# microsoft/NOTSOFAR1-Challenge

Hardware: AMD Instinct MI355X
Metric: CSS real-time-factor (sep. audio sec/wall sec) on 7-ch 16 kHz (higher is better)
Workload: dtype f32 (float32 operands on v_mfma_f32_32x32x2_f32 in every Linear layer, attention product and transform: the reference's own operand precision; MVDR covariance / solve f64)

## Files before the change

notsofar1-challenge_amd/csrc/encoder.hip:

```cpp
#include "kernels.hpp"
#include "split_f16.hpp"
#include "wave.hpp"

namespace css {

typedef float f32x16 __attribute__((ext_vector_type(16)));
typedef _Float16 f16x8 __attribute__((ext_vector_type(8)));

template <int NV>
__device__ __forceinline__ float ln_centre(float4 (&v)[NV]) {
    constexpr int D = 256 * NV;
    float s = 0.f;
#pragma unroll
    for (int i = 0; i < NV; ++i) s += (v[i].x + v[i].y) + (v[i].z + v[i].w);
    const float mean = wave_sum_dpp(s) * (1.0f / D);
    float q = 0.f;
#pragma unroll
    for (int i = 0; i < NV; ++i) {
        v[i].x -= mean; v[i].y -= mean; v[i].z -= mean; v[i].w -= mean;
        q += (v[i].x * v[i].x + v[i].y * v[i].y) + (v[i].z * v[i].z + v[i].w * v[i].w);
    }
    return 1.0f / sqrtf(wave_sum_dpp(q) * (1.0f / D) + 1e-5f);
}

#ifndef CSS_LN_ROWS
#define CSS_LN_ROWS 4
#endif
constexpr int LN_ROWS = CSS_LN_ROWS;
template <int NV, int MODE>
__global__ __launch_bounds__(64 * LN_ROWS) void layernorm_kernel(const float* __restrict__ x, float* __restrict__ y,
                                                        float* __restrict__ ys, const float* __restrict__ w,
                                                        const float* __restrict__ b, const float* __restrict__ pw,
                                                        int rows) {
    constexpr int D = 256 * NV;
    const int row = blockIdx.x * LN_ROWS + (threadIdx.x >> 6);
    if (row >= rows) return;
    const int lane = threadIdx.x & 63;
    const float4* xr = reinterpret_cast<const float4*>(x + (int64_t)row * D);
    float4 v[NV];
#pragma unroll
    for (int i = 0; i < NV; ++i) v[i] = xr[lane + 64 * i];
    const float rstd = ln_centre(v);
    float p0 = 0.f, p1 = 0.f, p2 = 0.f, p3 = 0.f;
    if (MODE == 2) { p0 = pw[0]; p1 = pw[1]; p2 = pw[2]; p3 = pw[3]; }
    float4* yr = reinterpret_cast<float4*>(y + (int64_t)row * D);
    _Float16* ysr = reinterpret_cast<_Float16*>(ys + (int64_t)row * D);
#pragma unroll
    for (int i = 0; i < NV; ++i) {
        const float4 g = reinterpret_cast<const float4*>(w)[lane + 64 * i];
        const float4 be = reinterpret_cast<const float4*>(b)[lane + 64 * i];
        float o[4] = {v[i].x * rstd * g.x + be.x, v[i].y * rstd * g.y + be.y, v[i].z * rstd * g.z + be.z,
                      v[i].w * rstd * g.w + be.w};
#pragma unroll
        for (int e = 0; e < 4; ++e) {
            if (MODE == 1) o[e] = fmaxf(o[e], 0.f);
            if (MODE == 2) o[e] = (p0 * o[e] + p1) * (1.0f / (1.0f + expf(-(p2 * o[e] + p3))));
        }
        if (y) yr[lane + 64 * i] = make_float4(o[0], o[1], o[2], o[3]);
        if (ys) split_store4(ysr, 4 * (lane + 64 * i), o[0], o[1], o[2], o[3]);
    }
}

template <int NV>
__global__ __launch_bounds__(64 * LN_ROWS) void layernorm2_kernel(const float* __restrict__ x, float* __restrict__ y,
                                                         const float* __restrict__ w1, const float* __restrict__ b1,
                                                         float* __restrict__ z, float* __restrict__ zs,
                                                         const float* __restrict__ w2, const float* __restrict__ b2,
                                                         int rows) {
    constexpr int D = 256 * NV;
    const int row = blockIdx.x * LN_ROWS + (threadIdx.x >> 6);
    if (row >= rows) return;
    const int lane = threadIdx.x & 63;
    const float4* xr = reinterpret_cast<const float4*>(x + (int64_t)row * D);
    float4 v[NV];
#pragma unroll
    for (int i = 0; i < NV; ++i) v[i] = xr[lane + 64 * i];
#pragma unroll
    for (int pass = 0; pass < 2; ++pass) {
        const float rstd = ln_centre(v);
        const float* w = pass ? w2 : w1;
        const float* b = pass ? b2 : b1;
        float* yo = pass ? z : y;
#pragma unroll
        for (int i = 0; i < NV; ++i) {
            const float4 g = reinterpret_cast<const float4*>(w)[lane + 64 * i];
            const float4 be = reinterpret_cast<const float4*>(b)[lane + 64 * i];
            v[i] = make_float4(v[i].x * rstd * g.x + be.x, v[i].y * rstd * g.y + be.y, v[i].z * rstd * g.z + be.z,
                               v[i].w * rstd * g.w + be.w);
            if (yo) reinterpret_cast<float4*>(yo + (int64_t)row * D)[lane + 64 * i] = v[i];
            if (pass && zs)
                split_store4(reinterpret_cast<_Float16*>(zs + (int64_t)row * D), 4 * (lane + 64 * i), v[i].x, v[i].y, v[i].z, v[i].w);
        }
    }
}

void launch_layernorm2(const float* x, float* y, const float* w1, const float* b1, float* z, float* z_split,
                       const float* w2, const float* b2, int rows, int D, hipStream_t s) {
    const dim3 grid((rows + LN_ROWS - 1) / LN_ROWS), block(64 * LN_ROWS);
    switch (D) {
        case 256: hipLaunchKernelGGL((layernorm2_kernel<1>), grid, block, 0, s, x, y, w1, b1, z, z_split, w2, b2, rows); break;
        case 512: hipLaunchKernelGGL((layernorm2_kernel<2>), grid, block, 0, s, x, y, w1, b1, z, z_split, w2, b2, rows); break;
        case 768: hipLaunchKernelGGL((layernorm2_kernel<3>), grid, block, 0, s, x, y, w1, b1, z, z_split, w2, b2, rows); break;
        case 1024: hipLaunchKernelGGL((layernorm2_kernel<4>), grid, block, 0, s, x, y, w1, b1, z, z_split, w2, b2, rows); break;
        default: break;
    }
}

template <int MODE>
static void launch_ln_mode(const float* x, float* y, float* ys, const float* w, const float* b, const float* pw,
                           int rows, int D, hipStream_t s) {
    const dim3 grid((rows + LN_ROWS - 1) / LN_ROWS), block(64 * LN_ROWS);
    switch (D) {
        case 256: hipLaunchKernelGGL((layernorm_kernel<1, MODE>), grid, block, 0, s, x, y, ys, w, b, pw, rows); break;
        case 512: hipLaunchKernelGGL((layernorm_kernel<2, MODE>), grid, block, 0, s, x, y, ys, w, b, pw, rows); break;
        case 768: hipLaunchKernelGGL((layernorm_kernel<3, MODE>), grid, block, 0, s, x, y, ys, w, b, pw, rows); break;
        case 1024: hipLaunchKernelGGL((layernorm_kernel<4, MODE>), grid, block, 0, s, x, y, ys, w, b, pw, rows); break;
        default: break;
    }
}

void launch_layernorm(const float* x, float* y, float* y_split, const float* w, const float* b, int rows, int D,
                      int relu, hipStream_t s) {
    if (relu) launch_ln_mode<1>(x, y, y_split, w, b, nullptr, rows, D, s);
    else launch_ln_mode<0>(x, y, y_split, w, b, nullptr, rows, D, s);
}

void launch_ln_glu(const float* x, float* z, const float* w, const float* b, const float* pw, int rows, int D,
                   hipStream_t s) {
    launch_ln_mode<2>(x, z, nullptr, w, b, pw, rows, D, s);
}

template <int TAPS, int RUN>
__global__ __launch_bounds__(256) void dwconv_kernel(const float* __restrict__ z, float* __restrict__ h,
                                                     const float* __restrict__ wt, const float* __restrict__ dwb,
                                                     const float* __restrict__ alpha, const float* __restrict__ beta,
                                                     const float* __restrict__ pw, int T, int D, int runs_per_seg) {
    constexpr int PAD = (TAPS - 1) / 2;
    const int ch = blockIdx.x * 256 + threadIdx.x;
    if (ch >= D) return;
    const int seg = blockIdx.y / runs_per_seg, run = blockIdx.y % runs_per_seg;
    const int t0 = run * RUN;
    const float* zs = z + (int64_t)seg * T * D + ch;
    float wk[TAPS];
#pragma clang loop unroll(full)
    for (int k = 0; k < TAPS; ++k) wk[k] = wt[k * D + ch];
    float acc[RUN];
#pragma clang loop unroll(full)
    for (int j = 0; j < RUN; ++j) acc[j] = 0.f;
#pragma clang loop unroll(full)
    for (int p = 0; p < RUN + TAPS - 1; ++p) {
        const int t = t0 + p - PAD;
        const float v = (t >= 0 && t < T) ? zs[(int64_t)t * D] : 0.f;
#pragma clang loop unroll(full)
        for (int j = (p - (TAPS - 1) > 0 ? p - (TAPS - 1) : 0); j <= (p < RUN - 1 ? p : RUN - 1); ++j)
            acc[j] = fmaf(wk[p - j], v, acc[j]);
    }
    const float bb = dwb[ch], al = alpha[ch], be = beta[ch], w2 = pw[4], c2 = pw[5];
    float* hs = h + (int64_t)seg * T * D + ch;
#pragma unroll
    for (int j = 0; j < RUN; ++j) {
        const int t = t0 + j;
        if (t < T) {
            const float y = fmaxf((acc[j] + bb) * al + be, 0.f);
            hs[(int64_t)t * D] += w2 * y + c2;
        }
    }
}

void launch_dwconv(const float* z, float* h, const float* dw_wt, const float* dw_b, const float* bn_alpha,
                   const float* bn_beta, const float* pw, int nseg, int T, int D, int taps, hipStream_t s) {
    constexpr int RUN = 31;
    const int runs = (T + RUN - 1) / RUN;
    const dim3 grid((D + 255) / 256, nseg * runs), block(256);
    if (taps == 33)
        hipLaunchKernelGGL((dwconv_kernel<33, RUN>), grid, block, 0, s, z, h, dw_wt, dw_b, bn_alpha, bn_beta, pw, T, D, runs);
    else if (taps == 31)
        hipLaunchKernelGGL((dwconv_kernel<31, RUN>), grid, block, 0, s, z, h, dw_wt, dw_b, bn_alpha, bn_beta, pw, T, D, runs);
    else if (taps == 17)
        hipLaunchKernelGGL((dwconv_kernel<17, RUN>), grid, block, 0, s, z, h, dw_wt, dw_b, bn_alpha, bn_beta, pw, T, D, runs);
}

template <int NV, int TAPS, int RUN, int HV>
__global__ __launch_bounds__(256 * NV * HV) void conv_module_kernel(const float* __restrict__ x_in, float* __restrict__ x_out,
                                                              const float* __restrict__ lnw, const float* __restrict__ lnb,
                                                              const float* __restrict__ pw, const float* __restrict__ wt,
                                                              const float* __restrict__ dwb, const float* __restrict__ alpha,
                                                              const float* __restrict__ beta,
                                                              const float* __restrict__ ln2w, const float* __restrict__ ln2b,
                                                              float* __restrict__ z, float* __restrict__ zs, int T, int runs_per_seg) {
    constexpr int D = 256 * NV, PAD = (TAPS - 1) / 2, ROWS = RUN + TAPS - 1, NW = 4 * NV * HV, JH = (RUN + HV - 1) / HV;
    extern __shared__ __attribute__((aligned(16))) float tile[];
    const int item = css_xcd_item((int)blockIdx.x, (int)gridDim.x);
    const int seg = item / runs_per_seg, run = item % runs_per_seg;
    const int t0 = run * RUN;
    const int wave = threadIdx.x >> 6, lane = threadIdx.x & 63;
    const float p0 = pw[0], p1 = pw[1], p2 = pw[2], p3 = pw[3];
    const int ch = threadIdx.x % D, j0 = (threadIdx.x / D) * JH;
    float wk[TAPS];
#pragma clang loop unroll(full)
    for (int k = 0; k < TAPS; ++k) wk[k] = wt[k * D + ch];
    const float bb = dwb[ch], al = alpha[ch], be_ = beta[ch], w2 = pw[4], c2 = pw[5];
    const float* xs = x_in + (int64_t)seg * T * D + ch;
    float xres[JH];
#pragma clang loop unroll(full)
    for (int j = 0; j < JH; ++j) xres[j] = xs[(int64_t)min(t0 + j0 + j, T - 1) * D];
    constexpr int RPW = (ROWS + NW - 1) / NW;
    float4 v[RPW][NV];
#pragma unroll
    for (int i = 0; i < RPW; ++i) {
        const int p = wave + i * NW, t = t0 + p - PAD;
        const bool ok = p < ROWS && t >= 0 && t < T;
        const float4* xr = reinterpret_cast<const float4*>(x_in + ((int64_t)seg * T + (ok ? t : 0)) * D);
#pragma unroll
        for (int j = 0; j < NV; ++j) v[i][j] = ok ? xr[lane + 64 * j] : make_float4(0.f, 0.f, 0.f, 0.f);
    }
#pragma unroll
    for (int i = 0; i < RPW; ++i) {
        const int p = wave + i * NW, t = t0 + p - PAD;
        if (p >= ROWS) break;
        float4* dst = reinterpret_cast<float4*>(tile + p * D);
        if (t < 0 || t >= T) {
#pragma unroll
            for (int j = 0; j < NV; ++j) dst[lane + 64 * j] = make_float4(0.f, 0.f, 0.f, 0.f);
            continue;
        }
        const float rstd = ln_centre(v[i]);
#pragma unroll
        for (int j = 0; j < NV; ++j) {
            const float4 g = reinterpret_cast<const float4*>(lnw)[lane + 64 * j];
            const float4 be = reinterpret_cast<const float4*>(lnb)[lane + 64 * j];
            float o[4] = {v[i][j].x * rstd * g.x + be.x, v[i][j].y * rstd * g.y + be.y, v[i][j].z * rstd * g.z + be.z,
                          v[i][j].w * rstd * g.w + be.w};
#pragma unroll
            for (int e = 0; e < 4; ++e) {
                const float z = p2 * o[e] + p3;
                o[e] = (p0 * o[e] + p1) * __builtin_amdgcn_rcpf(1.0f + __builtin_amdgcn_exp2f(z * -1.44269504088896341f));
            }
            dst[lane + 64 * j] = make_float4(o[0], o[1], o[2], o[3]);
        }
    }
    __syncthreads();
    float acc[JH];
#pragma clang loop unroll(full)
    for (int j = 0; j < JH; ++j) acc[j] = 0.f;
#pragma clang loop unroll(full)
    for (int pp = 0; pp < JH + TAPS - 1; ++pp) {
        const float zv = tile[min(j0 + pp, ROWS - 1) * D + ch];
#pragma clang loop unroll(full)
        for (int j = (pp - (TAPS - 1) > 0 ? pp - (TAPS - 1) : 0); j <= (pp < JH - 1 ? pp : JH - 1); ++j)
            acc[j] = fmaf(wk[pp - j], zv, acc[j]);
    }
    __syncthreads();
#pragma unroll
    for (int j = 0; j < JH; ++j) {
        const float y = fmaxf((acc[j] + bb) * al + be_, 0.f);
        if (j0 + j < RUN) tile[(j0 + j) * D + ch] = xres[j] + (w2 * y + c2);
    }
    __syncthreads();
    for (int j = wave; j < RUN && t0 + j < T; j += NW) {
        const int64_t row = (int64_t)seg * T + t0 + j;
        float4 r[NV];
#pragma unroll
        for (int i = 0; i < NV; ++i) {
            r[i] = reinterpret_cast<const float4*>(tile + j * D)[lane + 64 * i];
            reinterpret_cast<float4*>(x_out + row * D)[lane + 64 * i] = r[i];
        }
        if (!z && !zs) continue;
        const float rstd = ln_centre(r);
#pragma unroll
        for (int i = 0; i < NV; ++i) {
            const float4 g = reinterpret_cast<const float4*>(ln2w)[lane + 64 * i];
            const float4 be = reinterpret_cast<const float4*>(ln2b)[lane + 64 * i];
            const float4 o = make_float4(r[i].x * rstd * g.x + be.x, r[i].y * rstd * g.y + be.y, r[i].z * rstd * g.z + be.z,
                                         r[i].w * rstd * g.w + be.w);
            if (z) reinterpret_cast<float4*>(z + row * D)[lane + 64 * i] = o;
            if (zs) split_store4(reinterpret_cast<_Float16*>(zs + row * D), 4 * (lane + 64 * i), o.x, o.y, o.z, o.w);
        }
    }
}

bool launch_conv_module(const float* x_in, float* x_out, const float* ln_w, const float* ln_b, const float* pw,
                        const float* dw_wt, const float* dw_b, const float* bn_alpha, const float* bn_beta,
                        const float* ln2_w, const float* ln2_b, float* z, float* z_split, int nseg, int T,
                        int D, int taps, hipStream_t s) {
#ifndef CSS_CONV_RUN
#define CSS_CONV_RUN 31
#endif
    constexpr int RUN = CSS_CONV_RUN;
    if (taps != 33 || (D != 256 && D != 512)) return false;
    const int runs = (T + RUN - 1) / RUN;
    const size_t lds = (size_t)(RUN + 32) * D * sizeof(float);
    const void* fn = D == 512 ? reinterpret_cast<const void*>(&conv_module_kernel<2, 33, RUN, 2>)
                              : reinterpret_cast<const void*>(&conv_module_kernel<1, 33, RUN, 2>);
    if (hipFuncSetAttribute(fn, hipFuncAttributeMaxDynamicSharedMemorySize, 160 * 1024) != hipSuccess) {
        (void)hipGetLastError();
        return false;
    }
    if (D == 512)
        hipLaunchKernelGGL((conv_module_kernel<2, 33, RUN, 2>), dim3(nseg * runs), dim3(1024), lds, s, x_in, x_out, ln_w, ln_b, pw, dw_wt,
                           dw_b, bn_alpha, bn_beta, ln2_w, ln2_b, z, z_split, T, runs);
    else
        hipLaunchKernelGGL((conv_module_kernel<1, 33, RUN, 2>), dim3(nseg * runs), dim3(512), lds, s, x_in, x_out, ln_w, ln_b, pw, dw_wt,
                           dw_b, bn_alpha, bn_beta, ln2_w, ln2_b, z, z_split, T, runs);
    return true;
}

template <int NJT, bool QKS, bool FRAG, int W>
__global__ __launch_bounds__(64 * W, (NJT <= 7 ? 2 : 1)) void relpos_attn_kernel(const float* __restrict__ qkv, const float* __restrict__ qkf,
                                                         const float* __restrict__ pe,
                                                         float* __restrict__ ctx, int T, int D, int maxlen,
                                                         int split_out, int heads, int n_items) {
    constexpr int DK = 64;
    constexpr int LDR = 98;
    const int wv = W > 1 ? __builtin_amdgcn_readfirstlane((int)(threadIdx.x >> 6)) : 0;
    __shared__ __attribute__((aligned(16))) float lds_all[W][32 * LDR];
    float (&lds)[32 * LDR] = lds_all[wv];
    const int item = css_xcd_item((int)blockIdx.x, (int)gridDim.x) * W + wv;
    if (item >= n_items) return;
    const int qt = item % NJT, head = (item / NJT) % heads, seg = item / (NJT * heads);
    const int lane = threadIdx.x & 63, c = lane & 31, h = lane >> 5;
    const int ld = 3 * D;
    const float* qb = qkv + (int64_t)seg * T * ld + head * DK;
    const float* kb = qb + D;
    const float* vb = qb + 2 * D;
    const int i0 = qt * 32;
    const int iq = min(i0 + c, T - 1);

    float4 q[8];
#define CSS_ATT_LOAD8(dst, rowptr)                                                                      \
    _Pragma("unroll") for (int ch = 0; ch < 8; ++ch)                                                    \
        dst[ch] = *reinterpret_cast<const float4*>((rowptr) + (QKS ? ((ch >> 2) * 32 + ((ch >> 1) & 1) * 8 + (ch & 1) * 16) : 8 * ch) + 4 * h);
    const float4* qkt = reinterpret_cast<const float4*>(qkf) +
                        ((int64_t)(seg * heads + head) * NJT) * (2 * 8 * 64) + lane;
    if constexpr (FRAG) {
#pragma unroll
        for (int ch = 0; ch < 8; ++ch) q[ch] = qkt[(qt * 2 + 0) * 512 + ch * 64];
    } else {
        CSS_ATT_LOAD8(q, qb + (int64_t)iq * ld)
    }

    const int rel0 = i0 - (T - 1);
    auto pe_tile = [&](int rt) { return pe + ((int64_t)(qt + rt) * 8 * 64 + lane) * 4; };
    auto k_row = [&](int jt) { return kb + (int64_t)min(jt * 32 + c, T - 1) * ld; };
    (void)rel0; (void)maxlen;

    constexpr int RT0 = NJT;
    constexpr int NPRO = NJT >= 2 ? 3 : 2;
    constexpr int NI = NJT >= 2 ? NJT - 2 : 0;
    constexpr int NS = NPRO + NJT + NI;
    auto step_rt = [](int s_) {
        if (s_ < NPRO) return RT0 - s_;
        const int u_ = s_ - NPRO;
        return (u_ < 2 * NI && (u_ & 1)) ? RT0 - 3 - (u_ >> 1) : -1;
    };
    auto step_jt = [](int s_) {
        const int u_ = s_ - NPRO;
        return u_ < 2 * NI ? (u_ >> 1) : NI + (u_ - 2 * NI);
    };
#define CSS_ATT_LOAD_STEP(dst, s_)                                                                         \
    {                                                                                                      \
        if (step_rt(s_) >= 0) {                                                                            \
            const float4* pt_ = reinterpret_cast<const float4*>(pe_tile(step_rt(s_)));                     \
            _Pragma("unroll") for (int ch = 0; ch < 8; ++ch) dst[ch] = pt_[ch * 64];                       \
        } else if constexpr (FRAG) {                                                                       \
            _Pragma("unroll") for (int ch = 0; ch < 8; ++ch) dst[ch] = qkt[(step_jt(s_) * 2 + 1) * 512 + ch * 64]; \
        } else {                                                                                           \
            CSS_ATT_LOAD8(dst, k_row(step_jt(s_)))                                                         \
        }                                                                                                  \
    }
    constexpr int NTB = 2;
    float4 tb[NTB][8];
    f32x16 S[NJT];
    int step = 0;
#define CSS_ATT_LOAD_CH(dst, s_, ch)                                                                       \
    {                                                                                                      \
        if (step_rt(s_) >= 0) dst[ch] = reinterpret_cast<const float4*>(pe_tile(step_rt(s_)))[(ch) * 64];  \
        else if constexpr (FRAG) dst[ch] = qkt[(step_jt(s_) * 2 + 1) * 512 + (ch) * 64];                   \
        else dst[ch] = *reinterpret_cast<const float4*>(k_row(step_jt(s_)) + (QKS ? (((ch) >> 2) * 32 + (((ch) >> 1) & 1) * 8 + ((ch) & 1) * 16) : 8 * (ch)) + 4 * h); \
    }
#define CSS_ATT_STEP(acc)                                                                                  \
    {                                                                                                      \
        __builtin_amdgcn_sched_barrier(0);                                                                 \
        _Pragma("unroll") for (int r = 0; r < 16; ++r) acc[r] = 0.f;                                       \
        f32x16 cor_ = {0};                                                                                 \
        _Pragma("unroll") for (int ch = 0; ch < 8; ++ch) {                                                 \
            if (step + NTB - 1 < NS) { CSS_ATT_LOAD_CH(tb[(step + NTB - 1) % NTB], min(step + NTB - 1, NS - 1), ch) } \
            const float4 s4_ = tb[step % NTB][ch];                                                         \
            if constexpr (QKS) {    \
                if (ch & 1) {                                                                              \
                    const f16x8 sh_ = __builtin_bit_cast(f16x8, tb[step % NTB][ch - 1]), sl_ = __builtin_bit_cast(f16x8, s4_); \
                    const f16x8 qh_ = __builtin_bit_cast(f16x8, q[ch - 1]), ql_ = __builtin_bit_cast(f16x8, q[ch]);         \
                    acc = __builtin_amdgcn_mfma_f32_32x32x16_f16(sh_, qh_, acc, 0, 0, 0);                  \
                    cor_ = __builtin_amdgcn_mfma_f32_32x32x16_f16(sh_, ql_, cor_, 0, 0, 0);                \
                    cor_ = __builtin_amdgcn_mfma_f32_32x32x16_f16(sl_, qh_, cor_, 0, 0, 0);                \
                    __builtin_amdgcn_sched_barrier(0);                                                     \
                }                                                                                          \
            } else {                                                                                       \
                acc = __builtin_amdgcn_mfma_f32_32x32x2f32(s4_.x, q[ch].x, acc, 0, 0, 0);                  \
                acc = __builtin_amdgcn_mfma_f32_32x32x2f32(s4_.y, q[ch].y, acc, 0, 0, 0);                  \
                acc = __builtin_amdgcn_mfma_f32_32x32x2f32(s4_.z, q[ch].z, acc, 0, 0, 0);                  \
                acc = __builtin_amdgcn_mfma_f32_32x32x2f32(s4_.w, q[ch].w, acc, 0, 0, 0);                  \
                __builtin_amdgcn_sched_barrier(0);                                                         \
            }                                                                                              \
        }                                                                                                  \
        if constexpr (QKS) acc += cor_ * SPLIT_LO_INV;                                                     \
        __builtin_amdgcn_sched_barrier(0);                                                                 \
        ++step;                                                                                            \
    }
#define CSS_ATT_RING_WRITE(acc, rt)                                                          \
    {                                                                                        \
        const int slot_ = (((rt) % 3) + 3) % 3;                                              \
        _Pragma("unroll") for (int r = 0; r < 16; ++r)                                       \
            lds[c * LDR + slot_ * 32 + (r & 3) + 8 * (r >> 2) + 4 * h] = acc[r];             \
    }
    CSS_ATT_LOAD_STEP(tb[0], 0)
    if constexpr (NTB > 2) { CSS_ATT_LOAD_STEP(tb[1], 1) }
#pragma unroll
    for (int u = 0; u < NPRO; ++u) {
        const int rt = RT0 - u;
        f32x16 acc;
        CSS_ATT_STEP(acc)
        CSS_ATT_RING_WRITE(acc, rt)
    }
    float mx = -INFINITY;
    const int base_c = c + (T - 1) - 4 * h;
    const int m0 = base_c >= 0 ? base_c % 96 : 0;
    const float* ringc = lds + c * LDR;
#pragma unroll
    for (int jt = 0; jt < NJT; ++jt) {
        const int rt_new = RT0 - 3 - jt;
        CSS_ATT_STEP(S[jt])
#pragma unroll
        for (int r = 0; r < 16; ++r) {
            const int K = jt * 32 + (r & 3) + 8 * (r >> 2);
            float bpos, sc;
            if (jt < NJT - 1) {
                const unsigned t = (unsigned)(m0 - K % 96);
                bpos = ringc[min(t, t + 96u)];
                sc = S[jt][r] + bpos;
            } else {
                const int rr = max(base_c - K, 0);
                bpos = ringc[((rr >> 5) % 3) * 32 + (rr & 31)];
                sc = S[jt][r] + bpos;
                sc = K + 4 * h < T ? sc : -INFINITY;
            }
            S[jt][r] = sc;
            mx = fmaxf(mx, sc);
        }
        if (rt_new >= 0) {
            f32x16 acc;
            CSS_ATT_STEP(acc)
            CSS_ATT_RING_WRITE(acc, rt_new)
        }
    }
    mx = fmaxf(mx, __shfl_xor(mx, 32));
    const float c1 = 0.125f * 1.44269504088896341f, mc = mx * c1;
    float sum = 0.f;
#pragma unroll
    for (int jt = 0; jt < NJT; ++jt) {
#pragma unroll
        for (int r = 0; r < 16; ++r) {
            const float p = __builtin_amdgcn_exp2f(fmaf(S[jt][r], c1, -mc));
            S[jt][r] = p;
            sum += p;
        }
    }
    sum += __shfl_xor(sum, 32);
    const float inv = 1.0f / sum;
    __builtin_amdgcn_fence(__ATOMIC_RELEASE, "wavefront");
    __builtin_amdgcn_wave_barrier();

    constexpr int OLD = 65;
    if constexpr (QKS) {
        typedef __fp16 h4 __attribute__((__vector_size__(4 * sizeof(__fp16))));
        constexpr int VIMG = 32 * 32;
        constexpr int VLO = VIMG + 32;
        constexpr int VBUF = VLO + VIMG;
        static_assert(2 * VBUF * sizeof(_Float16) <= sizeof(lds), "V tile buffers must fit in the ring");
        _Float16* vlds = reinterpret_cast<_Float16*>(lds);
        float4 vr[4];
        const int vkey = lane >> 3, vpc = lane & 7;
#define CSS_ATT_VLOAD(g_)                                                                                          \
    _Pragma("unroll") for (int m = 0; m < 4; ++m) {                                                               \
        const int ju_ = ((g_) >> 1) * 32 + 8 * m + vkey;                                                          \
        const int row_ = ((g_) >> 1) < NJT - 1 ? ju_ : min(ju_, T - 1);                                           \
        vr[m] = *reinterpret_cast<const float4*>(vb + (int64_t)row_ * ld + ((g_) & 1) * 32 + 4 * vpc);            \
    }
#define CSS_ATT_VSTORE(g_)                                                                                         \
    _Pragma("unroll") for (int m = 0; m < 4; ++m)                                                                 \
        *reinterpret_cast<float4*>(vlds + ((g_) & 1) * VBUF + (vpc >> 2) * VLO + (8 * m + vkey) * 32 + (vpc & 3) * 8) = vr[m];
        const int tq = c >> 4, ti = c & 15;
        const int troff = (4 * h + (ti >> 2)) * 32 + 16 * tq + 4 * (ti & 3);
#define CSS_ATT_TR(g_, img_, kk_, eh_)                                                                             \
    __builtin_amdgcn_ds_read_tr16_b64_v4f16(reinterpret_cast<__attribute__((address_space(3))) h4*>(              \
        (__attribute__((address_space(3))) _Float16*)vlds + ((g_) & 1) * VBUF + (img_) * VLO + (16 * (kk_) + 8 * (eh_)) * 32 + troff))
        CSS_ATT_VLOAD(0)
        CSS_ATT_VSTORE(0)
        CSS_ATT_VLOAD(1)
        f32x16 o0 = {0}, o1 = {0}, cor0 = {0}, cor1 = {0};
#pragma unroll
        for (int jt = 0; jt < NJT; ++jt) {
            f16x8 ph[2], pl[2];
#pragma unroll
            for (int kk = 0; kk < 2; ++kk)
#pragma unroll
                for (int e = 0; e < 8; ++e) {
                    _Float16 a, b;
                    split_f16(S[jt][8 * kk + e], a, b);
                    ph[kk][e] = a;
                    pl[kk][e] = b;
                }
#pragma unroll
            for (int dt = 0; dt < 2; ++dt) {
                const int g = 2 * jt + dt;
                if (g + 1 < 2 * NJT) { CSS_ATT_VSTORE(g + 1) }
                if (g + 2 < 2 * NJT) { CSS_ATT_VLOAD(g + 2) }
#pragma unroll
                for (int kk = 0; kk < 2; ++kk) {
                    const h4 a0 = CSS_ATT_TR(g, 0, kk, 0), a1 = CSS_ATT_TR(g, 0, kk, 1);
                    const h4 b0 = CSS_ATT_TR(g, 1, kk, 0), b1 = CSS_ATT_TR(g, 1, kk, 1);
                    f16x8 vh, vl;
#pragma unroll
                    for (int e = 0; e < 4; ++e) {
                        vh[e] = (_Float16)a0[e]; vh[4 + e] = (_Float16)a1[e];
                        vl[e] = (_Float16)b0[e]; vl[4 + e] = (_Float16)b1[e];
                    }
                    if (dt == 0) {
                        o0 = __builtin_amdgcn_mfma_f32_32x32x16_f16(vh, ph[kk], o0, 0, 0, 0);
                        cor0 = __builtin_amdgcn_mfma_f32_32x32x16_f16(vh, pl[kk], cor0, 0, 0, 0);
                        cor0 = __builtin_amdgcn_mfma_f32_32x32x16_f16(vl, ph[kk], cor0, 0, 0, 0);
                    } else {
                        o1 = __builtin_amdgcn_mfma_f32_32x32x16_f16(vh, ph[kk], o1, 0, 0, 0);
                        cor1 = __builtin_amdgcn_mfma_f32_32x32x16_f16(vh, pl[kk], cor1, 0, 0, 0);
                        cor1 = __builtin_amdgcn_mfma_f32_32x32x16_f16(vl, ph[kk], cor1, 0, 0, 0);
                    }
                }
            }
        }
        o0 += cor0 * SPLIT_LO_INV;
        o1 += cor1 * SPLIT_LO_INV;
#pragma unroll
        for (int r = 0; r < 16; ++r) {
            const int d = (r & 3) + 8 * (r >> 2) + 4 * h;
            lds[c * OLD + d] = o0[r] * inv;
            lds[c * OLD + 32 + d] = o1[r] * inv;
        }
#undef CSS_ATT_VLOAD
#undef CSS_ATT_VSTORE
#undef CSS_ATT_TR
    } else {
    typedef float f32x2 __attribute__((ext_vector_type(2)));
    f32x2 vb2[2][16];
    const __amdgpu_buffer_rsrc_t rsv = __builtin_amdgcn_make_buffer_rsrc(const_cast<float*>(vb), 0, (int)(((int64_t)(T - 1) * ld + DK) * 4), 0x00020000);
    const int vvo = (4 * h * ld + 2 * c) * 4, ldb = ld * 4;
#define CSS_ATT_LOADV(jt_, r_) __builtin_bit_cast(f32x2, __builtin_amdgcn_raw_buffer_load_b64(rsv, vvo, ((jt_) * 32 + ((r_) & 3) + 8 * ((r_) >> 2)) * ldb, 0))
#pragma unroll
    for (int r = 0; r < 16; ++r) vb2[0][r] = CSS_ATT_LOADV(0, r);
    f32x16 oe = {0}, oo = {0};
#pragma unroll
    for (int jt = 0; jt < NJT; ++jt) {
        __builtin_amdgcn_sched_barrier(0);
#pragma unroll
        for (int r = 0; r < 16; ++r) {
            if (jt + 1 < NJT) vb2[(jt + 1) & 1][r] = CSS_ATT_LOADV(jt + 1, r);
            oe = __builtin_amdgcn_mfma_f32_32x32x2f32(vb2[jt & 1][r].x, S[jt][r], oe, 0, 0, 0);
            oo = __builtin_amdgcn_mfma_f32_32x32x2f32(vb2[jt & 1][r].y, S[jt][r], oo, 0, 0, 0);
            __builtin_amdgcn_sched_barrier(0);
        }
    }
#pragma unroll
    for (int r = 0; r < 16; ++r) {
        const int d = 2 * ((r & 3) + 8 * (r >> 2) + 4 * h);
        lds[c * OLD + d] = oe[r] * inv;
        lds[c * OLD + d + 1] = oo[r] * inv;
    }
#undef CSS_ATT_LOADV
    }
    __builtin_amdgcn_fence(__ATOMIC_RELEASE, "wavefront");
    __builtin_amdgcn_wave_barrier();
    {
        const int d4 = (lane & 15) * 4;
        float* ob = ctx + ((int64_t)seg * T + i0) * D;
#pragma unroll
        for (int k = 0; k < 8; ++k) {
            const int il = (lane >> 4) + 4 * k;
            if (i0 + il >= T) continue;
            const float* src = lds + il * OLD + d4;
            const float v0 = src[0], v1 = src[1], v2 = src[2], v3 = src[3];
            if (split_out)
                split_store4(reinterpret_cast<_Float16*>(ob + (int64_t)il * D), head * DK + d4, v0, v1, v2, v3);
            else
                *reinterpret_cast<float4*>(ob + (int64_t)il * D + head * DK + d4) = make_float4(v0, v1, v2, v3);
        }
    }
}

__global__ __launch_bounds__(256) void relpos_attn_long_kernel(const float* __restrict__ qkv, const float* __restrict__ pe,
                                                               float* __restrict__ ctx, int T, int D, int maxlen, int split_out,
                                                               int heads, int nq) {
    constexpr int DK = 64;
    extern __shared__ __attribute__((aligned(16))) float att_lds[];
    const int qtiles = (T + nq - 1) / nq;
    const int item = blockIdx.x;
    const int qt = item % qtiles, head = (item / qtiles) % heads, seg = item / (qtiles * heads);
    const int i0 = qt * nq, nv = min(nq, T - i0);
    float* qs = att_lds;
    float* ss = qs + nq * DK;
    const int tid = threadIdx.x;
    const int64_t ld = 3 * (int64_t)D;
    const float* base = qkv + (int64_t)seg * T * ld + head * DK;
    for (int e = tid; e < nv * DK; e += 256) qs[e] = base[(int64_t)(i0 + e / DK) * ld + (e % DK)];
    __syncthreads();
    const int sub = tid & 3, kq = tid >> 2;
    auto quad_sum = [](float v) {
        v = dpp_add<0xB1>(v);
        return dpp_add<0x4E>(v);
    };
    auto load_row = [&](const float* rowp, float (&row)[16]) {
#pragma unroll
        for (int m = 0; m < 4; ++m) {
            const float4 v = *reinterpret_cast<const float4*>(rowp + 16 * m + 4 * sub);
            row[4 * m] = v.x; row[4 * m + 1] = v.y; row[4 * m + 2] = v.z; row[4 * m + 3] = v.w;
        }
    };
    auto dots4 = [&](int i, const float (&row)[16], float (&acc)[4]) {
#pragma unroll
        for (int k = 0; k < 4; ++k) acc[k] = 0.f;
#pragma unroll
        for (int m = 0; m < 4; ++m)
#pragma unroll
            for (int k = 0; k < 4; ++k) {
                const float4 q = *reinterpret_cast<const float4*>(qs + min(i + k, nv - 1) * DK + 16 * m + 4 * sub);
                acc[k] = fmaf(q.x, row[4 * m], acc[k]); acc[k] = fmaf(q.y, row[4 * m + 1], acc[k]);
                acc[k] = fmaf(q.z, row[4 * m + 2], acc[k]); acc[k] = fmaf(q.w, row[4 * m + 3], acc[k]);
            }
#pragma unroll
        for (int k = 0; k < 4; ++k) acc[k] = quad_sum(acc[k]);
    };
    for (int j0 = 0; j0 < T; j0 += 64) {
        const int j = j0 + kq;
        float row[16];
        load_row(base + (int64_t)min(j, T - 1) * ld + D, row);
        for (int i = 0; i < nv; i += 4) {
            float acc[4];
            dots4(i, row, acc);
            const float mine = sub == 0 ? acc[0] : sub == 1 ? acc[1] : sub == 2 ? acc[2] : acc[3];
            if (j < T && i + sub < nv) ss[(size_t)(i + sub) * T + j] = mine;
        }
    }
    __syncthreads();
    const int nu = nv + T - 1;
    for (int u0 = 0; u0 < nu; u0 += 64) {
        const int u = u0 + kq;
        const int rel = max(-maxlen, min(i0 - (T - 1) + u, maxlen - 1)) + maxlen;
        float row[16];
        load_row(pe + (int64_t)rel * DK, row);
        for (int i = 0; i < nv; i += 4) {
            float acc[4];
            dots4(i, row, acc);
            const float mine = sub == 0 ? acc[0] : sub == 1 ? acc[1] : sub == 2 ? acc[2] : acc[3];
            const int j = i + sub + T - 1 - u;
            if (u < nu && i + sub < nv && j >= 0 && j < T) ss[(size_t)(i + sub) * T + j] = (ss[(size_t)(i + sub) * T + j] + mine) * 0.125f;
        }
    }
    __syncthreads();
    const int wave = tid >> 6, lane = tid & 63;
    for (int i = wave; i < nv; i += 4) {
        float* row = ss + (size_t)i * T;
        float mx = -INFINITY;
        for (int j = lane; j < T; j += 64) mx = fmaxf(mx, row[j]);
        mx = wave_max_shfl(mx);
        float sum = 0.f;
        for (int j = lane; j < T; j += 64) { const float e = expf(row[j] - mx); row[j] = e; sum += e; }
        sum = wave_sum_dpp(sum);
        const float inv = 1.0f / sum;
        for (int j = lane; j < T; j += 64) row[j] *= inv;
    }
    __syncthreads();
    {
        const int d = tid & 63, ig = tid >> 6;
        constexpr int MAXQ = 4;
        float acc[MAXQ] = {0.f, 0.f, 0.f, 0.f};
        const float* vb = base + 2 * D + d;
#pragma unroll 8
        for (int j = 0; j < T; ++j) {
            const float v = vb[(int64_t)j * ld];
#pragma unroll
            for (int k = 0; k < MAXQ; ++k) {
                const int i = ig + 4 * k;
                if (i < nv) acc[k] = fmaf(ss[(size_t)i * T + j], v, acc[k]);
            }
        }
        float* ob = ctx + ((int64_t)seg * T + i0) * D;
#pragma unroll
        for (int k = 0; k < MAXQ; ++k) {
            const int i = ig + 4 * k;
            if (i >= nv) continue;
            if (split_out) split_store(reinterpret_cast<_Float16*>(ob + (int64_t)i * D), head * DK + d, acc[k]);
            else ob[(int64_t)i * D + head * DK + d] = acc[k];
        }
    }
}

bool launch_relpos_attention_long(const float* qkv, const float* pe, float* ctx, int nseg, int T, int D, int H, int maxlen,
                                  int split_out, hipStream_t s) {
    if (D != H * 64) return false;
    int nq = 16;
    auto bytes = [&](int n) { return ((size_t)n * 64 + (size_t)n * T) * sizeof(float); };
    while (nq > 1 && bytes(nq) > 52 * 1024) nq >>= 1;
    if (bytes(nq) > 150 * 1024) return false;
    if (bytes(nq) > 65536 && hipFuncSetAttribute(reinterpret_cast<const void*>(relpos_attn_long_kernel),
                                                 hipFuncAttributeMaxDynamicSharedMemorySize, (int)bytes(nq)) != hipSuccess)
        return false;
    const unsigned qtiles = (unsigned)((T + nq - 1) / nq);
    hipLaunchKernelGGL(relpos_attn_long_kernel, dim3(qtiles * (unsigned)H * (unsigned)nseg), dim3(256), bytes(nq), s, qkv, pe, ctx, T, D,
                       maxlen, split_out, H, nq);
    return true;
}

__global__ __launch_bounds__(256) void pe_fragments_kernel(const float* __restrict__ pe, float* __restrict__ frag, int T,
                                                           int maxlen, int ntiles, int split) {
    const int i = blockIdx.x * 256 + threadIdx.x;
    if (i >= ntiles * 8 * 64) return;
    const int lane = i & 63, ch = (i >> 6) & 7, m = i >> 9;
    const int c = lane & 31, h = lane >> 5;
    int prow = 32 * m - (T - 1) + c;
    prow = max(-maxlen, min(prow, maxlen - 1)) + maxlen;
    const int off = (split ? ((ch >> 2) * 32 + ((ch >> 1) & 1) * 8 + (ch & 1) * 16) : 8 * ch) + 4 * h;
    reinterpret_cast<float4*>(frag)[i] = *reinterpret_cast<const float4*>(pe + (int64_t)prow * 64 + off);
}

void launch_pe_fragments(const float* pe, float* frag, int T, int maxlen, int split, hipStream_t s) {
    const int ntiles = pe_fragment_tiles(T);
    hipLaunchKernelGGL(pe_fragments_kernel, dim3((ntiles * 8 * 64 + 255) / 256), dim3(256), 0, s, pe, frag, T, maxlen, ntiles, split);
}

#ifndef CSS_ATT_WAVES
#define CSS_ATT_WAVES 4
#endif
void launch_relpos_attention(const float* qkv, const float* qk_frag, const float* pe_frag, float* ctx, int nseg, int T, int D,
                             int H, int maxlen, int qk_split, int split_out, hipStream_t s) {
    const int qtiles = (T + 31) / 32;
    const int n_items = qtiles * H * nseg;
#define CSS_ATT_LAUNCH(n, w)                                                                                                 \
    {                                                                                                                        \
        const dim3 grid((unsigned)((n_items + (w) - 1) / (w))), block(64 * (w));                                              \
        if (qk_split && qk_frag) hipLaunchKernelGGL((relpos_attn_kernel<n, true, true, w>), grid, block, 0, s, qkv, qk_frag, pe_frag, ctx, T, D, maxlen, split_out, H, n_items);  \
        else if (qk_split) hipLaunchKernelGGL((relpos_attn_kernel<n, true, false, w>), grid, block, 0, s, qkv, qk_frag, pe_frag, ctx, T, D, maxlen, split_out, H, n_items);  \
        else hipLaunchKernelGGL((relpos_attn_kernel<n, false, false, w>), grid, block, 0, s, qkv, qk_frag, pe_frag, ctx, T, D, maxlen, split_out, H, n_items);          \
    }
#define CSS_ATT_CASE(n) case n: CSS_ATT_LAUNCH(n, (n <= 7 ? CSS_ATT_WAVES : 1)) break;
    switch (qtiles) {
        CSS_ATT_CASE(1) CSS_ATT_CASE(2) CSS_ATT_CASE(3) CSS_ATT_CASE(4)
        CSS_ATT_CASE(5) CSS_ATT_CASE(6) CSS_ATT_CASE(7) CSS_ATT_CASE(8)
        CSS_ATT_CASE(9) CSS_ATT_CASE(10) CSS_ATT_CASE(11) CSS_ATT_CASE(12)
        CSS_ATT_CASE(13) CSS_ATT_CASE(14) CSS_ATT_CASE(15) CSS_ATT_CASE(16)
        default: break;
    }
#undef CSS_ATT_CASE
#undef CSS_ATT_LAUNCH
}

}
```

Baseline: 7360.

## Interleave ring writes, bias adds and softmax exp under attention MFMA chains

For the non-QKS f32 path, the relpos attention kernel is rewritten as a compile-time unrolled schedule. Ring-buffer LDS writes of positional-score tiles, the relative-bias gather/add with running max, and the first V-tile loads are slotted between the MFMA instructions of the following step. The softmax exp for tile jt+1 and the final sum reduction are likewise moved inside the P·V MFMA loop, and the ring is widened to 130 columns with a duplicated slot so the bias gathers avoid wraparound. This aims to hide VALU/LDS latency behind matrix instructions, at the cost of higher register pressure and more complex code. Optional s_memtime probes are added under a compile-time flag.

```diff
diff --git a/notsofar1-challenge_amd/csrc/encoder.hip b/notsofar1-challenge_amd/csrc/encoder.hip
--- a/notsofar1-challenge_amd/csrc/encoder.hip
+++ b/notsofar1-challenge_amd/csrc/encoder.hip
@@ -1,6 +1,8 @@
 #include "kernels.hpp"
 #include "split_f16.hpp"
 #include "wave.hpp"
+#include <type_traits>
+#include <utility>
 
 namespace css {
 
@@ -305,18 +307,60 @@
     return true;
 }
 
+#ifdef CSS_ATT_PROBE
+__device__ unsigned long long* css_att_probe_buf;
+void set_att_probe(unsigned long long* buf) { (void)hipMemcpyToSymbol(HIP_SYMBOL(css_att_probe_buf), &buf, sizeof(buf)); }
+#define CSS_ATT_STAMP(k)                                                                                   \
+    {                                                                                                      \
+        __builtin_amdgcn_sched_barrier(0);                                                                 \
+        unsigned long long t_;                                                                             \
+        asm volatile("s_memtime %0\n\ts_waitcnt lgkmcnt(0)" : "=s"(t_) :: "memory");                       \
+        pr_sum[k] += t_ - pr_t;                                                                            \
+        pr_t = t_;                                                                                         \
+        __builtin_amdgcn_sched_barrier(0);                                                                 \
+    }
+#define CSS_ATT_GAP(k) pr_gap = (k);
+#else
+#define CSS_ATT_STAMP(k)
+#define CSS_ATT_GAP(k)
+#endif
+
+template <class F, int... I>
+__device__ __forceinline__ void static_for_seq(F&& f, std::integer_sequence<int, I...>) { (f(std::integral_constant<int, I>{}), ...); }
+template <int N, class F>
+__device__ __forceinline__ void static_for(F&& f) { static_for_seq(f, std::make_integer_sequence<int, N>{}); }
+
+template <int NJT>
+struct AttSchedule {
+    static constexpr int RT0 = NJT, NPRO = NJT >= 2 ? 3 : 2, NI = NJT >= 2 ? NJT - 2 : 0, NS = NPRO + NJT + NI;
+    static constexpr int rt(int s) {
+        if (s < NPRO) return RT0 - s;
+        const int u = s - NPRO;
+        return (u < 2 * NI && (u & 1)) ? RT0 - 3 - (u >> 1) : -1;
+    }
+    static constexpr int jt(int s) {
+        const int u = s - NPRO;
+        return u < 2 * NI ? (u >> 1) : NI + (u - 2 * NI);
+    }
+};
+
 template <int NJT, bool QKS, bool FRAG, int W>
 __global__ __launch_bounds__(64 * W, (NJT <= 7 ? 2 : 1)) void relpos_attn_kernel(const float* __restrict__ qkv, const float* __restrict__ qkf,
                                                          const float* __restrict__ pe,
                                                          float* __restrict__ ctx, int T, int D, int maxlen,
                                                          int split_out, int heads, int n_items) {
     constexpr int DK = 64;
-    constexpr int LDR = 98;
+    constexpr int LDR = QKS ? 98 : 130;
     const int wv = W > 1 ? __builtin_amdgcn_readfirstlane((int)(threadIdx.x >> 6)) : 0;
     __shared__ __attribute__((aligned(16))) float lds_all[W][32 * LDR];
     float (&lds)[32 * LDR] = lds_all[wv];
     const int item = css_xcd_item((int)blockIdx.x, (int)gridDim.x) * W + wv;
     if (item >= n_items) return;
+#ifdef CSS_ATT_PROBE
+    unsigned long long pr_sum[8] = {0, 0, 0, 0, 0, 0, 0, 0}, pr_t;
+    int pr_gap = 0;
+    asm volatile("s_memtime %0\n\ts_waitcnt lgkmcnt(0)" : "=s"(pr_t) :: "memory");
+#endif
     const int qt = item % NJT, head = (item / NJT) % heads, seg = item / (NJT * heads);
     const int lane = threadIdx.x & 63, c = lane & 31, h = lane >> 5;
     const int ld = 3 * D;
@@ -345,18 +389,11 @@
     (void)rel0; (void)maxlen;
 
     constexpr int RT0 = NJT;
-    constexpr int NPRO = NJT >= 2 ? 3 : 2;
-    constexpr int NI = NJT >= 2 ? NJT - 2 : 0;
-    constexpr int NS = NPRO + NJT + NI;
-    auto step_rt = [](int s_) {
-        if (s_ < NPRO) return RT0 - s_;
-        const int u_ = s_ - NPRO;
-        return (u_ < 2 * NI && (u_ & 1)) ? RT0 - 3 - (u_ >> 1) : -1;
-    };
-    auto step_jt = [](int s_) {
-        const int u_ = s_ - NPRO;
-        return u_ < 2 * NI ? (u_ >> 1) : NI + (u_ - 2 * NI);
-    };
+    using Sch = AttSchedule<NJT>;
+    [[maybe_unused]] constexpr int NPRO = Sch::NPRO, NI = Sch::NI, NS = Sch::NS;
+    static_assert(Sch::RT0 == RT0, "one schedule");
+    auto step_rt = [](int s_) { return Sch::rt(s_); };
+    auto step_jt = [](int s_) { return Sch::jt(s_); };
 #define CSS_ATT_LOAD_STEP(dst, s_)                                                                         \
     {                                                                                                      \
         if (step_rt(s_) >= 0) {                                                                            \
@@ -380,6 +417,7 @@
     }
 #define CSS_ATT_STEP(acc)                                                                                  \
     {                                                                                                      \
+        CSS_ATT_STAMP(pr_gap)                                                                              \
         __builtin_amdgcn_sched_barrier(0);                                                                 \
         _Pragma("unroll") for (int r = 0; r < 16; ++r) acc[r] = 0.f;                                       \
         f32x16 cor_ = {0};                                                                                 \
@@ -405,6 +443,7 @@
         }                                                                                                  \
         if constexpr (QKS) acc += cor_ * SPLIT_LO_INV;                                                     \
         __builtin_amdgcn_sched_barrier(0);                                                                 \
+        CSS_ATT_STAMP(1)                                                                                   \
         ++step;                                                                                            \
     }
 #define CSS_ATT_RING_WRITE(acc, rt)                                                          \
@@ -413,23 +452,108 @@
         _Pragma("unroll") for (int r = 0; r < 16; ++r)                                       \
             lds[c * LDR + slot_ * 32 + (r & 3) + 8 * (r >> 2) + 4 * h] = acc[r];             \
     }
+    float mx = -INFINITY;
+    const int base_c = c + (T - 1) - 4 * h;
+    const int m0 = base_c >= 0 ? base_c % 96 : 0;
+    const float* ringc = lds + c * LDR;
+    typedef float f32x2 __attribute__((ext_vector_type(2)));
+    [[maybe_unused]] f32x2 vb2[2][16];
+    const __amdgpu_buffer_rsrc_t rsv = __builtin_amdgcn_make_buffer_rsrc(const_cast<float*>(vb), 0, (int)(((int64_t)(T - 1) * ld + DK) * 4), 0x00020000);
+    const int vvo = (4 * h * ld + 2 * c) * 4, ldb = ld * 4;
+#define CSS_ATT_LOADV(jt_, r_) __builtin_bit_cast(f32x2, __builtin_amdgcn_raw_buffer_load_b64(rsv, vvo, ((jt_) * 32 + ((r_) & 3) + 8 * ((r_) >> 2)) * ldb, 0))
+    [[maybe_unused]] f32x16 racc[2];
+    [[maybe_unused]] float bp[8];
+    [[maybe_unused]] const float* rp = ringc;
+    [[maybe_unused]] auto under = [&](auto sc_, auto mc_) __attribute__((always_inline)) {
+        constexpr int s = decltype(sc_)::value, m = decltype(mc_)::value;
+        if constexpr (s > 0) {
+            constexpr int prt = Sch::rt(s - 1), pjt = Sch::jt(s - 1);
+            if constexpr (prt >= 0) {
+                if constexpr (m >= 8 && m < 24 && (m & 3) == 0) {
+                    static_for<4>([&](auto i_) __attribute__((always_inline)) {
+                        constexpr int r = m - 8 + decltype(i_)::value;
+                        constexpr int col = (prt % 3) * 32 + (r & 3) + 8 * (r >> 2);
+                        lds[c * LDR + col + 4 * h] = racc[(s - 1) & 1][r];
+                        if constexpr (prt % 3 == 0) lds[c * LDR + 96 + col + 4 * h] = racc[(s - 1) & 1][r];
+                    });
+                }
+            } else {
+                if constexpr (m == 4) {
+                    const int t = m0 - (32 * pjt) % 96;
+                    int b27 = (t >= 27 ? t : t + 96) - 27;
+                    asm volatile("" : "+v"(b27));
+                    rp = ringc + b27;
+                }
+                if constexpr (m >= 6 && m < 22) bp[(m - 6) & 7] = rp[27 - (((m - 6) & 3) + 8 * ((m - 6) >> 2))];
+                if constexpr (m >= 10 && m < 26) {
+                    const float sc = S[pjt][m - 10] + bp[(m - 10) & 7];
+                    S[pjt][m - 10] = sc;
+                    mx = fmaxf(mx, sc);
+                }
+            }
+        }
+        if constexpr (s == NS - 1 && (m & 1) == 0) vb2[0][m >> 1] = CSS_ATT_LOADV(0, m >> 1);
+    };
+    [[maybe_unused]] auto step_f32 = [&](auto sc_, f32x16& acc) __attribute__((always_inline)) {
+        constexpr int s = decltype(sc_)::value;
+        CSS_ATT_STAMP(pr_gap)
+        __builtin_amdgcn_sched_barrier(0);
+#pragma unroll
+        for (int r = 0; r < 16; ++r) acc[r] = 0.f;
+        static_for<8>([&](auto ch_) __attribute__((always_inline)) {
+            constexpr int ch = decltype(ch_)::value;
+            if constexpr (s + 1 < NS) { CSS_ATT_LOAD_CH(tb[(s + 1) % NTB], s + 1, ch) }
+            const float4 s4_ = tb[s % NTB][ch];
+            acc = __builtin_amdgcn_mfma_f32_32x32x2f32(s4_.x, q[ch].x, acc, 0, 0, 0);
+            under(sc_, std::integral_constant<int, 4 * ch + 0>{});
+            __builtin_amdgcn_sched_barrier(0);
+            acc = __builtin_amdgcn_mfma_f32_32x32x2f32(s4_.y, q[ch].y, acc, 0, 0, 0);
+            under(sc_, std::integral_constant<int, 4 * ch + 1>{});
+            __builtin_amdgcn_sched_barrier(0);
+            acc = __builtin_amdgcn_mfma_f32_32x32x2f32(s4_.z, q[ch].z, acc, 0, 0, 0);
+            under(sc_, std::integral_constant<int, 4 * ch + 2>{});
+            __builtin_amdgcn_sched_barrier(0);
+            acc = __builtin_amdgcn_mfma_f32_32x32x2f32(s4_.w, q[ch].w, acc, 0, 0, 0);
+            under(sc_, std::integral_constant<int, 4 * ch + 3>{});
+            __builtin_amdgcn_sched_barrier(0);
+        });
+        CSS_ATT_STAMP(1)
+    };
     CSS_ATT_LOAD_STEP(tb[0], 0)
     if constexpr (NTB > 2) { CSS_ATT_LOAD_STEP(tb[1], 1) }
+    if constexpr (!QKS) {
+        static_for<NS>([&](auto sc_) __attribute__((always_inline)) {
+            constexpr int s = decltype(sc_)::value;
+            if constexpr (Sch::rt(s) >= 0) {
+                step_f32(sc_, racc[s & 1]);
+                CSS_ATT_GAP(2)
+            } else {
+                step_f32(sc_, S[Sch::jt(s)]);
+                CSS_ATT_GAP(s < NS - 1 ? 3 : 4)
+            }
+        });
+#pragma unroll
+        for (int r = 0; r < 16; ++r) {
+            const int K = (NJT - 1) * 32 + (r & 3) + 8 * (r >> 2);
+            const int rr = max(base_c - K, 0);
+            const float sc = S[NJT - 1][r] + ringc[((rr >> 5) % 3) * 32 + (rr & 31)];
+            S[NJT - 1][r] = K + 4 * h < T ? sc : -INFINITY;
+            mx = fmaxf(mx, S[NJT - 1][r]);
+        }
+    } else {
 #pragma unroll
     for (int u = 0; u < NPRO; ++u) {
         const int rt = RT0 - u;
         f32x16 acc;
         CSS_ATT_STEP(acc)
+        CSS_ATT_GAP(2)
         CSS_ATT_RING_WRITE(acc, rt)
     }
-    float mx = -INFINITY;
-    const int base_c = c + (T - 1) - 4 * h;
-    const int m0 = base_c >= 0 ? base_c % 96 : 0;
-    const float* ringc = lds + c * LDR;
 #pragma unroll
     for (int jt = 0; jt < NJT; ++jt) {
         const int rt_new = RT0 - 3 - jt;
         CSS_ATT_STEP(S[jt])
+        CSS_ATT_GAP(jt < NJT - 1 ? 3 : 4)
 #pragma unroll
         for (int r = 0; r < 16; ++r) {
             const int K = jt * 32 + (r & 3) + 8 * (r >> 2);
@@ -450,14 +574,17 @@
         if (rt_new >= 0) {
             f32x16 acc;
             CSS_ATT_STEP(acc)
+            CSS_ATT_GAP(2)
             CSS_ATT_RING_WRITE(acc, rt_new)
         }
     }
+    }
     mx = fmaxf(mx, __shfl_xor(mx, 32));
+    CSS_ATT_STAMP(pr_gap)
     const float c1 = 0.125f * 1.44269504088896341f, mc = mx * c1;
-    float sum = 0.f;
-#pragma unroll
-    for (int jt = 0; jt < NJT; ++jt) {
+    float sum = 0.f, inv = 0.f;
+#pragma unroll
+    for (int jt = 0; jt < (QKS ? NJT : 1); ++jt) {
 #pragma unroll
         for (int r = 0; r < 16; ++r) {
             const float p = __builtin_amdgcn_exp2f(fmaf(S[jt][r], c1, -mc));
@@ -465,10 +592,13 @@
             sum += p;
         }
     }
-    sum += __shfl_xor(sum, 32);
-    const float inv = 1.0f / sum;
+    if constexpr (QKS) {
+        sum += __shfl_xor(sum, 32);
+        inv = 1.0f / sum;
+    }
     __builtin_amdgcn_fence(__ATOMIC_RELEASE, "wavefront");
     __builtin_amdgcn_wave_barrier();
+    CSS_ATT_STAMP(5)
 
     constexpr int OLD = 65;
     if constexpr (QKS) {
@@ -549,25 +679,27 @@
 #undef CSS_ATT_VSTORE
 #undef CSS_ATT_TR
     } else {
-    typedef float f32x2 __attribute__((ext_vector_type(2)));
-    f32x2 vb2[2][16];
-    const __amdgpu_buffer_rsrc_t rsv = __builtin_amdgcn_make_buffer_rsrc(const_cast<float*>(vb), 0, (int)(((int64_t)(T - 1) * ld + DK) * 4), 0x00020000);
-    const int vvo = (4 * h * ld + 2 * c) * 4, ldb = ld * 4;
-#define CSS_ATT_LOADV(jt_, r_) __builtin_bit_cast(f32x2, __builtin_amdgcn_raw_buffer_load_b64(rsv, vvo, ((jt_) * 32 + ((r_) & 3) + 8 * ((r_) >> 2)) * ldb, 0))
-#pragma unroll
-    for (int r = 0; r < 16; ++r) vb2[0][r] = CSS_ATT_LOADV(0, r);
     f32x16 oe = {0}, oo = {0};
-#pragma unroll
-    for (int jt = 0; jt < NJT; ++jt) {
+    static_for<NJT>([&](auto jt_) __attribute__((always_inline)) {
+        constexpr int jt = decltype(jt_)::value;
         __builtin_amdgcn_sched_barrier(0);
-#pragma unroll
-        for (int r = 0; r < 16; ++r) {
-            if (jt + 1 < NJT) vb2[(jt + 1) & 1][r] = CSS_ATT_LOADV(jt + 1, r);
+        static_for<16>([&](auto r_) __attribute__((always_inline)) {
+            constexpr int r = decltype(r_)::value;
+            if constexpr (jt + 1 < NJT) vb2[(jt + 1) & 1][r] = CSS_ATT_LOADV(jt + 1, r);
             oe = __builtin_amdgcn_mfma_f32_32x32x2f32(vb2[jt & 1][r].x, S[jt][r], oe, 0, 0, 0);
             oo = __builtin_amdgcn_mfma_f32_32x32x2f32(vb2[jt & 1][r].y, S[jt][r], oo, 0, 0, 0);
+            if constexpr (jt + 1 < NJT) {
+                const float p = __builtin_amdgcn_exp2f(fmaf(S[jt + 1][r], c1, -mc));
+                S[jt + 1][r] = p;
+                sum += p;
+            } else if constexpr (r == 1) {
+                sum += __shfl_xor(sum, 32);
+            } else if constexpr (r == 5) {
+                inv = 1.0f / sum;
+            }
             __builtin_amdgcn_sched_barrier(0);
-        }
-    }
+        });
+    });
 #pragma unroll
     for (int r = 0; r < 16; ++r) {
         const int d = 2 * ((r & 3) + 8 * (r >> 2) + 4 * h);
@@ -576,6 +708,7 @@
     }
 #undef CSS_ATT_LOADV
     }
+    CSS_ATT_STAMP(6)
     __builtin_amdgcn_fence(__ATOMIC_RELEASE, "wavefront");
     __builtin_amdgcn_wave_barrier();
     {
@@ -593,6 +726,14 @@
                 *reinterpret_cast<float4*>(ob + (int64_t)il * D + head * DK + d4) = make_float4(v0, v1, v2, v3);
         }
     }
+#ifdef CSS_ATT_PROBE
+    asm volatile("s_waitcnt vmcnt(0)" ::: "memory");
+    CSS_ATT_STAMP(7)
+    if (lane == 0 && css_att_probe_buf) {
+#pragma unroll
+        for (int k = 0; k < 8; ++k) css_att_probe_buf[(int64_t)item * 8 + k] = pr_sum[k];
+    }
+#endif
 }
 
 __global__ __launch_bounds__(256) void relpos_attn_long_kernel(const float* __restrict__ qkv, const float* __restrict__ pe,
```

New measurement: 7432 (median of 6 runs). Within noise of the previous version (+1.0%).
